# JARVIS-MoCap/JARVIS-HybridNet

Hardware: AMD Instinct MI355X
Metric: multi-view frames/s (12cam 1280x1024, 23kpt, 64^3 grid) (higher is better)
Workload: dtype f32; 1 GPU; BASELINE configs[2]: HybridNet 12-camera 1280x1024, 23 kpts, 64^3 grid, small/small; cameras=12, joints=23, grid=64, streams=3, parallelism=single GPU, 3 time batches in flight on 3 HIP streams, hipgraph=False

## Files before the change

include/jarvis_hip.h:

```cpp
#ifndef JARVIS_HIP_H
#define JARVIS_HIP_H
#include <stdint.h>

#ifdef __cplusplus
extern "C" {
#endif

#define JH_ABI_VERSION 4

const char* jh_last_error(void);
int jh_abi_version(void);

#define JH_PRECISION_DEFAULT (-1)
#define JH_PRECISION_F32 0
#define JH_PRECISION_BF16X3 1
#define JH_PRECISION_BF16X3_WIDE 2
int jh_set_precision(int mode);
int jh_get_precision(void);

typedef struct jh_params jh_params;
int jh_params_create(jh_params** out);
int jh_params_set(jh_params* p, const char* key, const float* host, int64_t numel);
void jh_params_destroy(jh_params* p);

// ... 152 lines not shown
int jh_predictor_set_spread(jh_predictor* pr, int on);
int jh_predictor_get_spread(jh_predictor* pr, float* cov_dev, float* peak_dev, float* mass_dev, void* stream);
int jh_predictor_debug_v2v(jh_predictor* pr, float* out_dev, void* stream);

#define JH_FRAME_SURFACE  4
#define JH_FRAME_SENSOR   5
int jh_predictor_forward_images(jh_predictor* pr, const void* const* images_host, int n_images, int format,
                                const jh_yuv_surface* yuv, const jh_sensor_surface* sensor, const uint8_t* mask_dev,
                                float* points_dev, float* conf_dev, int32_t* valid_dev, void* stream);

typedef struct jh_subjects_params {
  int32_t max_subjects, max_peaks, nms_radius, min_views;
  float min_peak, max_error_px;
} jh_subjects_params;
int jh_subjects_params_check(const jh_subjects_params* params);
int jh_op_center_peaks(const float* heat_dev, int n, int hh, int wh, int cp, const jh_subjects_params* params,
                       float* peaks_dev, int32_t* count_dev, void* stream);
int jh_op_associate_subjects(const float* peaks_dev, int t, int cams, const float* cam_dev, const float* intr_dev,
                             const float* dist_dev, int calib_per_frame, const uint8_t* mask_dev, float sx2, float sy2,
                             const jh_subjects_params* params, float* centers_dev, int32_t* views_dev,
                             int32_t* members_dev, float* error_dev, void* stream);
int jh_predictor_detect_subjects(jh_predictor* pr, const void* frames_dev, const void* const* images_host, int n_images,
                                 int format, const jh_yuv_surface* yuv, const jh_sensor_surface* sensor,
                                 const uint8_t* mask_dev, const jh_subjects_params* params, float* centers_dev,
                                 int32_t* views_dev, int32_t* members_dev, float* error_dev,
                                 float* peaks_dev , void* stream);

typedef struct jh_track_params {
  int32_t max_subjects;
  int32_t max_missed;
// ... 136 lines not shown
```

jarvis-hybridnet_amd/_native.py:

```python
import ctypes
import math
import os
from typing import NamedTuple

import torch

_HERE = os.path.dirname(os.path.abspath(__file__))
LIB_PATH = os.environ.get("JH_LIBRARY_PATH") or os.path.join(_HERE, "libjarvis_hip.so")
_lib = None

c_void_p, c_int, c_float, c_int64 = ctypes.c_void_p, ctypes.c_int, ctypes.c_float, ctypes.c_int64
c_char_p = ctypes.c_char_p


class PredictorConfig(ctypes.Structure):
    _fields_ = [("num_cameras", ctypes.c_int32), ("num_joints", ctypes.c_int32),
                ("center_size", ctypes.c_int32), ("bbox", ctypes.c_int32),
                ("roi_cube_size", c_float), ("grid_spacing", c_float),
                ("center_model", ctypes.c_int32), ("kp_model", ctypes.c_int32),
                ("img_h", ctypes.c_int32), ("img_w", ctypes.c_int32),
                ("time_batch", ctypes.c_int32), ("time_batch_3d", ctypes.c_int32),
                ("cam_lo", ctypes.c_int32),
                ("cam_n", ctypes.c_int32), ("mean", c_float * 3), ("std", c_float * 3),
                ("precision", ctypes.c_int32)]
# ... 147 lines not shown
    "jh_predictor_forward_masked": (c_int, [c_void_p, c_void_p, c_int, c_void_p, c_void_p, c_void_p, c_void_p,
                                            c_void_p]),
    "jh_predictor_forward_images": (c_int, [c_void_p, ctypes.POINTER(c_void_p), c_int, c_int,
                                            ctypes.POINTER(YuvSurfaceStruct), ctypes.POINTER(SensorSurfaceStruct),
                                            c_void_p, c_void_p, c_void_p, c_void_p, c_void_p]),
    "jh_predictor2d_forward_images": (c_int, [c_void_p, ctypes.POINTER(c_void_p), c_int, c_int,
                                              ctypes.POINTER(YuvSurfaceStruct), ctypes.POINTER(SensorSurfaceStruct),
                                              c_void_p, c_void_p, c_void_p, c_void_p]),
    "jh_predictor_stage_keypoints_masked": (c_int, [c_void_p, c_void_p, c_int, c_void_p, c_void_p, c_void_p,
                                                    c_void_p]),
    "jh_predictor_stage_3d_masked": (c_int, [c_void_p, c_void_p, c_int, c_void_p, c_void_p, c_void_p, c_void_p,
                                             c_void_p]),
    "jh_predictor_debug_mask": (c_int, [c_void_p, c_void_p, c_void_p, c_void_p]),
    "jh_predictor_views2d": (c_int, [c_void_p, c_void_p, c_int] + [c_void_p] * 8),
    "jh_subjects_params_check": (c_int, [ctypes.POINTER(SubjectsParamsStruct)]),
    "jh_op_center_peaks": (c_int, [c_void_p, c_int, c_int, c_int, c_int, ctypes.POINTER(SubjectsParamsStruct), c_void_p,
                                   c_void_p, c_void_p]),
    "jh_op_associate_subjects": (c_int, [c_void_p, c_int, c_int, c_void_p, c_void_p, c_void_p, c_int, c_void_p,
                                         c_float, c_float, ctypes.POINTER(SubjectsParamsStruct), c_void_p, c_void_p,
                                         c_void_p, c_void_p, c_void_p]),
    "jh_predictor_detect_subjects": (c_int, [c_void_p, c_void_p, ctypes.POINTER(c_void_p), c_int, c_int,
                                             ctypes.POINTER(YuvSurfaceStruct), ctypes.POINTER(SensorSurfaceStruct),
                                             c_void_p, ctypes.POINTER(SubjectsParamsStruct), c_void_p, c_void_p,
                                             c_void_p, c_void_p, c_void_p, c_void_p]),
    "jh_track_params_check": (c_int, [ctypes.POINTER(TrackParamsStruct)]),
    "jh_op_track_reset": (c_int, [c_void_p, c_void_p]),
    "jh_op_track_subjects": (c_int, [c_void_p, c_void_p, c_void_p, c_void_p, c_int, c_int,
                                     ctypes.POINTER(TrackParamsStruct)] + [c_void_p] * 10),
    "jh_joints3d_params_check": (c_int, [ctypes.POINTER(Joints3dParamsStruct)]),
    "jh_op_joint_peaks_refine": (c_int, [c_void_p, c_int, c_int, c_int, c_int, c_void_p, c_int, c_int, c_void_p,
# ... 460 lines not shown
```

jarvis-hybridnet_amd/csrc/api.hip:

```cpp
#include <cstring>
#include <memory>
#include "../../include/jarvis_hip.h"
#include <cstdlib>
#include "nets.h"
#include "bifpn_node.h"
#include "views2d.h"
#include "subjects.h"
#include "joints3d.h"
#include "tracks.h"

namespace jh {
static thread_local std::string g_err;
void set_error(const std::string& msg) { g_err = msg; }
}

using namespace jh;

struct jh_params { ParamMap map; };
struct jh_efftrack { EffTrackPlan plan; };
struct jh_v2v { V2VPlan plan; };

namespace {

struct Scratch {
// ... 616 lines not shown
  pr->J = cfg->num_joints; pr->Jp = cpad(cfg->num_joints);
  pr->B = cfg->bbox; pr->Hh = cfg->bbox / 2; pr->hs = cfg->bbox / 2 + 2;
  pr->G = (int)(cfg->roi_cube_size / cfg->grid_spacing);
  pr->Gh = pr->G / 2;
  JH_REQUIRE(pr->T >= 1 && pr->C >= 1 && pr->C <= 64, "time batch / camera count");
  JH_REQUIRE(cfg->cam_lo >= 0 && cfg->cam_n >= 1 && cfg->cam_lo + cfg->cam_n <= pr->C, "camera range");
  JH_REQUIRE(pr->G % 4 == 0, "ROI_CUBE_SIZE / GRID_SPACING must be a multiple of 4");
  const int N = pr->T * pr->Cloc;
  const NodeBatchClass node_class = pr->T >= 8 ? NodeBatchClass::AtLeast8 : NodeBatchClass::Below8;
  const int norm_kb = node_class == NodeBatchClass::AtLeast8 && JH_ENV_KNOB("JH_NODE_ROWS") != 0 ? 64 : 0;
  PlanSetup setup;
  if (setup.init(&pr->cfg, node_class, norm_kb)) return 1;
  if (center_params) {
    pr->center = setup.efftrack();
    if (pr->center->build(center_params->map, "", cfg->center_model, 1, N, cfg->center_size,
                          cfg->center_size)) return 1;
  }
  pr->kp = setup.efftrack();
  if (pr->kp->build(hybrid_params->map, "effTrack.", cfg->kp_model, pr->J, N, pr->B, pr->B)) return 1;
  pr->v2v.reset(new V2VPlan());
  pr->v2v->precision = setup.precision;
  pr->v2v->norm_block_kb = norm_kb;
  if (pr->v2v->build(hybrid_params->map, "v2vNet.", pr->J, pr->T3, pr->G)) return 1;
  auto& m = pr->mem;
  const int T = pr->T, C = pr->C;
  if (m.get(reinterpret_cast<void**>(&pr->cam), (size_t)C * 12 * sizeof(float))) return 1;
  if (m.get(reinterpret_cast<void**>(&pr->intr), (size_t)C * 9 * sizeof(float))) return 1;
  if (m.get(reinterpret_cast<void**>(&pr->dist), (size_t)C * 5 * sizeof(float))) return 1;
  if (m.get(reinterpret_cast<void**>(&pr->det_all), (size_t)T * C * 3 * sizeof(float))) return 1;
  if (m.get(reinterpret_cast<void**>(&pr->c3f), (size_t)T * 3 * sizeof(float))) return 1;
  for (auto& cs : pr->cset) {
// ... 826 lines not shown

extern "C" {

int jh_predictor2d_create(const jh_params* center_params, const jh_params* kp_params,
                          const jh_predictor_config* cfg, jh_predictor2d** out) {
  JH_REQUIRE(center_params && kp_params && cfg && out, "bad argument");
  std::unique_ptr<jh_predictor2d> pr(new jh_predictor2d());
  pr->cfg = *cfg;
  pr->T = cfg->time_batch; pr->J = cfg->num_joints; pr->B = cfg->bbox;
  JH_REQUIRE(pr->T >= 1, "batch");
  JH_REQUIRE(cfg->img_w >= pr->B + 1 && cfg->img_h >= pr->B + 1, "image smaller than the bounding box");
  PlanSetup setup;
  if (setup.init(&pr->cfg, NodeBatchClass::ByLaunchSize, 0)) return 1;
  pr->center = setup.efftrack();
  if (pr->center->build(center_params->map, "", cfg->center_model, 1, pr->T, cfg->center_size,
                        cfg->center_size)) return 1;
  pr->kp = setup.efftrack();
  if (pr->kp->build(kp_params->map, "", cfg->kp_model, pr->J, pr->T, pr->B, pr->B)) return 1;
  if (pr->mem.get(reinterpret_cast<void**>(&pr->det), (size_t)pr->T * 3 * sizeof(float))) return 1;
  if (pr->mem.get(reinterpret_cast<void**>(&pr->chm), (size_t)pr->T * 2 * sizeof(int))) return 1;
  if (pr->mem.get(reinterpret_cast<void**>(&pr->valid), (size_t)pr->T * sizeof(int))) return 1;
  JH_CHECK_HIP(hipDeviceSynchronize());
  *out = pr.release();
  return 0;
}

void jh_predictor2d_destroy(jh_predictor2d* pr) { delete pr; }

static int forward2d_impl(jh_predictor2d* pr, const Call& call, int32_t* points_dev, float* conf_dev,
                          int32_t* valid_dev) {
  hipStream_t s = call.s;
// ... 221 lines not shown
               const float* w_host, const float* b_host, const float* x_dev, int n, int d, int h,
               int w, const float* gate_dev, int norm_act, float* y_dev, void* stream) {
  return op_conv_body(nd, kind, k, stride, pad, cin, cout, w_host, b_host, x_dev, n, d, h, w, gate_dev, norm_act,
                      nullptr, y_dev, static_cast<hipStream_t>(stream), "jh_op_conv");
}

int jh_op_conv_operand(int nd, int kind, int k, int stride, int pad, int cin, int cout,
                       const float* w_host, const float* b_host, const float* x_dev, int n, int d, int h,
                       int w, const float* gate_dev, const jh_op_operand* operand, float* y_dev, void* stream) {
  JH_REQUIRE(operand && w_host && x_dev && y_dev && n >= 1, "bad argument");
  JH_REQUIRE(operand->in_act >= ACT_NONE && operand->in_act <= ACT_SILU, "jh_op_conv_operand: in_act");
  JH_REQUIRE(operand->latency_class == 0 || operand->latency_class == 1, "jh_op_conv_operand: latency_class");
  JH_REQUIRE(!(gate_dev && operand->se_pool_host), "either a gate tensor or a gate recipe");
  return op_conv_body(nd, kind, k, stride, pad, cin, cout, w_host, b_host, x_dev, n, d, h, w, gate_dev, -1, operand,
                      y_dev, static_cast<hipStream_t>(stream), "jh_op_conv_operand");
}

int jh_op_se_gate(const double* pool_host, int n, int c, int squeeze, float inv_hw, const float* wr_host,
                  const float* br_host, const float* we_host, const float* be_host, float* gate_dev, void* stream) {
  hipStream_t s = static_cast<hipStream_t>(stream);
  JH_REQUIRE(gate_dev && n >= 1, "bad argument");
  Scratch sc;
  SeGate se;
  const int Cp = cpad(c);
  if (op_upload_se(sc, pool_host, n, c, Cp, squeeze, inv_hw, wr_host, br_host, we_host, be_host, &se)) return 1;
  float* gate = nullptr;
  if (sc.get(reinterpret_cast<void**>(&gate), (size_t)n * Cp * sizeof(float))) return 1;
  if (launch_se_gate(se.pool, n, c, Cp, squeeze, inv_hw, se.wr, se.br, se.we, se.be, gate, s)) return 1;
  JH_CHECK_HIP(hipMemcpy2DAsync(gate_dev, c * sizeof(float), gate, Cp * sizeof(float), c * sizeof(float), n,
                                hipMemcpyDeviceToDevice, s));
// ... 222 lines not shown
```

jarvis-hybridnet_amd/csrc/deconv_c1.hip:

```cpp
#include "jh_common.h"
#include "operand_load.h"

namespace jh {

constexpr int kDcTY = 8, kDcTX = 16, kDcPY = 10, kDcPX = 18;

__global__ __launch_bounds__(256) void deconv_c1_kernel(
    const float* __restrict__ x, const double* __restrict__ st, float inv_cnt, int in_act,
    const float* __restrict__ w , float* __restrict__ y, int H, int W, int Cp,
    int cout_p) {
  extern __shared__ __attribute__((aligned(16))) float sm[];
  const int S = Cp + 4;
  float* nrm = sm;
  float* tile = nrm + 2 * Cp;
  const int tid = threadIdx.x;
  const BlockId bid = xcd_block();
  const int tiles_x = (W + kDcTX - 1) / kDcTX;
  const int y0 = (bid.x / tiles_x) * kDcTY, x0 = (bid.x % tiles_x) * kDcTX;
  const int n = bid.y;
  const int q = Cp >> 2;

  for (int c = tid; c < Cp; c += 256) {
    float mean = 0.f, rstd = 1.f;
    if (st) {
      const NormCoef k = norm_coef_times_inv(st + ((size_t)n * Cp + c) * kStatW, inv_cnt);
      mean = k.mean;
      rstd = k.rstd;
    }
    nrm[c] = mean;
    nrm[Cp + c] = rstd;
  }
  __syncthreads();
  const float* xin = x + (size_t)n * H * W * Cp;
  {
    constexpr int NPX = kDcPY * kDcPX, ITERS = (NPX + 15) / 16, UB = ITERS;
    const int slot = tid >> 4;
   for (int cq0 = 0; cq0 < q; cq0 += 16) {
    const int lc4 = cq0 + (tid & 15);
    const bool cact = lc4 < q;
    float4 mu = make_float4(0.f, 0.f, 0.f, 0.f), rs = make_float4(1.f, 1.f, 1.f, 1.f);
    if (cact) {
      mu = *reinterpret_cast<const float4*>(nrm + lc4 * 4);
      rs = *reinterpret_cast<const float4*>(nrm + Cp + lc4 * 4);
    }
#pragma unroll
    for (int it0 = 0; it0 < ITERS; it0 += UB) {
      float4 v[UB];
      bool ok[UB];
#pragma unroll
      for (int u = 0; u < UB; ++u) {
        const int pix = (it0 + u) * 16 + slot;
        const int iy = y0 - 1 + pix / kDcPX, ix = x0 - 1 + pix % kDcPX;
        ok[u] = it0 + u < ITERS && pix < NPX && cact && iy >= 0 && iy < H && ix >= 0 && ix < W;
        v[u] = ok[u] ? *reinterpret_cast<const float4*>(xin + ((size_t)iy * W + ix) * Cp + lc4 * 4)
                     : make_float4(0.f, 0.f, 0.f, 0.f);
      }
#pragma unroll
      for (int u = 0; u < UB; ++u) {
        const int pix = (it0 + u) * 16 + slot;
        if (it0 + u < ITERS && pix < NPX && cact) {
          float4 x4 = v[u];
          if (ok[u]) x4 = act4(norm_sub4(x4, mu, rs), in_act);
          *reinterpret_cast<float4*>(tile + pix * S + lc4 * 4) = x4;
        }
      }
    }
   }
  }
  __syncthreads();

  const int py = __builtin_amdgcn_readfirstlane(tid >> 7);
  const int p = tid & 127;
  const int tm = p / kDcTX, tn = p % kDcTX;
  const int ra = py ? tm + 2 : tm + 1, ka = py ? 0 : 1;
  const int rb = py ? tm + 1 : tm, kb = py ? 2 : 3;
  const float* ta = tile + (ra * kDcPX + tn) * S;
  const float* tb = tile + (rb * kDcPX + tn) * S;
  const float* __restrict__ wa = w + ka * 4 * Cp;
  const float* __restrict__ wb = w + kb * 4 * Cp;
  float o0 = 0.f, o1 = 0.f;
  for (int c = 0; c < Cp; c += 4) {
    const float4 a0 = *reinterpret_cast<const float4*>(ta + c);
    const float4 a1 = *reinterpret_cast<const float4*>(ta + S + c);
    const float4 a2 = *reinterpret_cast<const float4*>(ta + 2 * S + c);
    const float4 b0 = *reinterpret_cast<const float4*>(tb + c);
    const float4 b1 = *reinterpret_cast<const float4*>(tb + S + c);
    const float4 b2 = *reinterpret_cast<const float4*>(tb + 2 * S + c);
    const float4 wa0 = *reinterpret_cast<const float4*>(wa + 0 * Cp + c);
    const float4 wa1 = *reinterpret_cast<const float4*>(wa + 1 * Cp + c);
    const float4 wa2 = *reinterpret_cast<const float4*>(wa + 2 * Cp + c);
    const float4 wa3 = *reinterpret_cast<const float4*>(wa + 3 * Cp + c);
    const float4 wb0 = *reinterpret_cast<const float4*>(wb + 0 * Cp + c);
    const float4 wb1 = *reinterpret_cast<const float4*>(wb + 1 * Cp + c);
    const float4 wb2 = *reinterpret_cast<const float4*>(wb + 2 * Cp + c);
    const float4 wb3 = *reinterpret_cast<const float4*>(wb + 3 * Cp + c);
#define JH_DOT4(acc, u, v) acc = fmaf(u.x, v.x, acc); acc = fmaf(u.y, v.y, acc); \
                           acc = fmaf(u.z, v.z, acc); acc = fmaf(u.w, v.w, acc);
    JH_DOT4(o0, a1, wa1) JH_DOT4(o0, a0, wa3) JH_DOT4(o0, b1, wb1) JH_DOT4(o0, b0, wb3)
    JH_DOT4(o1, a2, wa0) JH_DOT4(o1, a1, wa2) JH_DOT4(o1, b2, wb0) JH_DOT4(o1, b1, wb2)
#undef JH_DOT4
  }
  const int m = y0 + tm, nn = x0 + tn;
  if (m < H && nn < W) {
    float* dst = y + (((size_t)n * 2 * H + 2 * m + py) * 2 * W + 2 * nn) * cout_p;
    for (int o = 0; o < 2; ++o) {
      float* d = dst + o * cout_p;
      *reinterpret_cast<float4*>(d) = make_float4(o ? o1 : o0, 0.f, 0.f, 0.f);
      for (int c = 4; c < cout_p; c += 4) *reinterpret_cast<float4*>(d + c) = make_float4(0.f, 0.f, 0.f, 0.f);
    }
  }
}

int launch_deconv_c1(const Act& x, const double* stats, float inv_cnt, int in_act, const float* w,
                     const Act& y, hipStream_t s) {
  JH_REQUIRE(y.H == 2 * x.H && y.W == 2 * x.W && y.N == x.N && y.C == 1, "deconv_c1 shapes");
  const size_t lds = ((size_t)2 * x.Cp + (size_t)kDcPY * kDcPX * (x.Cp + 4)) * sizeof(float);
  JH_REQUIRE(lds <= 160 * 1024, "deconv_c1 tile does not fit LDS");
  static bool big = false;
  if (lds > 64 * 1024 && !big) {
    JH_CHECK_HIP(hipFuncSetAttribute(reinterpret_cast<const void*>(deconv_c1_kernel),
                                     hipFuncAttributeMaxDynamicSharedMemorySize, 160 * 1024));
    big = true;
  }
  const int tiles = ((x.H + kDcTY - 1) / kDcTY) * ((x.W + kDcTX - 1) / kDcTX);
  hipLaunchKernelGGL(deconv_c1_kernel, dim3(tiles, x.N), dim3(256), lds, s, x.p, stats, inv_cnt,
                     in_act, w, y.p, x.H, x.W, x.Cp, y.Cp);
  JH_CHECK_HIP(hipGetLastError());
  return 0;
}

}
```

jarvis-hybridnet_amd/csrc/geometry.hip:

```cpp
#include "jh_common.h"
#include "dlt.h"
#include "preprocess.h"
#include "views2d.h"
#include "subjects.h"
#include "nets.h"

namespace jh {

template <int SRC>
__global__ __launch_bounds__(256) void preprocess_resize_kernel(
    const void* __restrict__ frames, float* __restrict__ out, int N, int H, int W, int S,
    float sy, float sx, float3 mean, float3 stdv, const void* const* __restrict__ frames_cell, int per_image,
    SrcDesc<SRC> d) {
  if (frames_cell && !per_image) frames = *frames_cell;
  const size_t total = (size_t)N * S * S;
  for (size_t i = (size_t)blockIdx.x * blockDim.x + threadIdx.x; i < total;
       i += (size_t)gridDim.x * blockDim.x) {
    const int ox = (int)(i % S), oy = (int)((i / S) % S);
    int n = (int)(i / ((size_t)S * S));
    const void* base = image_base(frames, frames_cell, per_image, n);
    *reinterpret_cast<float4*>(out + i * 4) = resize_px<SRC>(base, n, oy, ox, H, W, sy, sx, mean, stdv, d);
  }
}

// ... 545 lines not shown
                         const unsigned char* mask, const float* pts3d, const Calib& cal, int* points2d,
                         float* conf2d, float* reproj, float* err, unsigned char* used, int T, int C, int J, int Jp,
                         int Hh, int Wh, int hw, hipStream_t s) {
  if (check_scan_shape(T * C, Hh, Wh, J, Jp)) return 1;
  if (calib_check(cal, C)) return 1;
  const ScanShape sh = joint_argmax_all_shape(T * C, Hh, Wh, Jp);
  hipLaunchKernelGGL(views2d_final_kernel, dim3(T * C), dim3(round_up(J, kWave)), 0, s, pmax, pidx, center_hm,
                     valid, mask, pts3d, cal.cam, cal.intr, cal.dist, cal.fs, points2d, conf2d, reproj, err, used, C, J,
                     Jp, sh.slices, Hh, Wh, hw);
  JH_CHECK_HIP(hipGetLastError());
  return 0;
}

__device__ __forceinline__ float softplus_f(float x) { return x > 20.f ? x : log1pf(expf(x)); }

constexpr int kSpreadSums = 10, kSpreadRound = 5;
__device__ __forceinline__ unsigned long long spread_key(float x, unsigned p) {
  const unsigned u = __float_as_uint(x);
  const unsigned k = (u & 0x80000000u) ? ~u : (u | 0x80000000u);
  return ((unsigned long long)k << 32) | (unsigned long long)(0xFFFFFFFFu - p);
}
__device__ __forceinline__ unsigned long long max_u64(unsigned long long a, unsigned long long b) {
  return a > b ? a : b;
}
__device__ __forceinline__ void spread_acc(double* s, float h, double di, double dj, double dk) {
  const double d = (double)h, hi = d * di, hj = d * dj, hk = d * dk;
  s[0] += d; s[1] += hi; s[2] += hj; s[3] += hk;
  s[4] += hi * di; s[5] += hi * dj; s[6] += hi * dk;
  s[7] += hj * dj; s[8] += hj * dk; s[9] += hk * dk;
}
// ... 1 lines not shown
template <bool SPREAD>
__global__ __launch_bounds__(256) void softargmax_partial_kernel(
    const float* __restrict__ x, double* __restrict__ partial, int* __restrict__ pmax,
    double* __restrict__ spart, unsigned long long* __restrict__ skey, int Gh, int Jp, int ppb) {
  extern __shared__ __attribute__((aligned(16))) float sm[];
  const int q = Jp >> 2, rows = 256 / q, tid = threadIdx.x;
  const bool active = tid < rows * q;
  const int c4 = tid % q, row = tid / q;
  const int t = blockIdx.y;
  const int P = Gh * Gh * Gh;
  const int p0 = blockIdx.x * ppb, p1 = min(P, p0 + ppb);
  float4 s0 = make_float4(0, 0, 0, 0), si = s0, sj = s0, sk = s0, mx = s0;
  [[maybe_unused]] double ds[SPREAD ? 4 : 1][SPREAD ? kSpreadSums : 1] = {};
  [[maybe_unused]] unsigned long long key[SPREAD ? 4 : 1] = {};
  if (active) {
    for (int p = p0 + row; p < p1; p += rows) {
      const float4 v = *reinterpret_cast<const float4*>(x + ((size_t)t * P + p) * Jp + c4 * 4);
      const float4 h = make_float4(softplus_f(v.x), softplus_f(v.y), softplus_f(v.z), softplus_f(v.w));
      const float fk = (float)(p % Gh), fj = (float)((p / Gh) % Gh), fi = (float)(p / (Gh * Gh));
      s0.x += h.x; s0.y += h.y; s0.z += h.z; s0.w += h.w;
      si.x += h.x * fi; si.y += h.y * fi; si.z += h.z * fi; si.w += h.w * fi;
      sj.x += h.x * fj; sj.y += h.y * fj; sj.z += h.z * fj; sj.w += h.w * fj;
      sk.x += h.x * fk; sk.y += h.y * fk; sk.z += h.z * fk; sk.w += h.w * fk;
      mx.x = fmaxf(mx.x, h.x); mx.y = fmaxf(mx.y, h.y); mx.z = fmaxf(mx.z, h.z); mx.w = fmaxf(mx.w, h.w);
      if constexpr (SPREAD) {
        const double di = (double)fi, dj = (double)fj, dk = (double)fk;
        spread_acc(ds[0], h.x, di, dj, dk);
        spread_acc(ds[1], h.y, di, dj, dk);
        spread_acc(ds[2], h.z, di, dj, dk);
        spread_acc(ds[3], h.w, di, dj, dk);
        key[0] = max_u64(key[0], spread_key(v.x, (unsigned)p));
        key[1] = max_u64(key[1], spread_key(v.y, (unsigned)p));
        key[2] = max_u64(key[2], spread_key(v.z, (unsigned)p));
        key[3] = max_u64(key[3], spread_key(v.w, (unsigned)p));
      }
    }
  }
  if (active) {
    float4* p = reinterpret_cast<float4*>(sm) + ((size_t)row * q + c4) * 5;
    p[0] = s0; p[1] = si; p[2] = sj; p[3] = sk; p[4] = mx;
  }
  __syncthreads();
  for (int i = tid; i < q * 4 * 5; i += 256) {
    const int comp = i & 3, v = (i >> 2) % 5, cq = (i >> 2) / 5;
    const int ch = cq * 4 + comp;
    if (v < 4) {
      float acc = 0.f;
      for (int r = 0; r < rows; ++r) acc += sm[(((size_t)r * q + cq) * 5 + v) * 4 + comp];
      exact_add(partial + (((size_t)t * Jp + ch) * 4 + v) * kLimbs, (double)acc);
    } else {
      float m = 0.f;
      for (int r = 0; r < rows; ++r) m = fmaxf(m, sm[(((size_t)r * q + cq) * 5 + v) * 4 + comp]);
      atomicMax(pmax + (size_t)t * Jp + ch, __float_as_int(m));
    }
  }
  if constexpr (SPREAD) {
    constexpr int W = kSpreadRound + 1;
    double* dm = reinterpret_cast<double*>(sm);
#pragma unroll
    for (int round = 0; round < kSpreadSums / kSpreadRound; ++round) {
      __syncthreads();
      if (active) {
#pragma unroll
// ... 96 lines not shown

int launch_softargmax(const float* x, const int* center3d, double* partial, int* pmax,
                      float* points, float* conf, float* heatmap_final, int T, int J, int Jp,
                      int Gh, float spacing, float roi, hipStream_t s, const SoftargmaxSpread* sp) {
  const int P = Gh * Gh * Gh;
  const int q = Jp / 4;
  JH_REQUIRE(q >= 1 && q <= 64 && J <= 256, "soft-argmax joint count");
  const int rows = 256 / q;
  const size_t pbytes = (size_t)T * Jp * 4 * kLimbs * sizeof(double), mbytes = (size_t)T * Jp * sizeof(int);
  if (reinterpret_cast<char*>(pmax) == reinterpret_cast<char*>(partial) + pbytes) {
    if (launch_zero(partial, pbytes + mbytes, s)) return 1;
  } else {
    if (launch_zero(partial, pbytes, s)) return 1;
    if (launch_zero(pmax, mbytes, s)) return 1;
  }
  const int ppb = rows * 8;
  dim3 grid((P + ppb - 1) / ppb, T);
  if (sp) {
    JH_REQUIRE(sp->sums && sp->key && sp->cov && sp->peak && sp->mass, "soft-argmax spread: null pointer");
    JH_REQUIRE(grid.x <= (1u << 13), "soft-argmax spread: more than 2^13 blocks per frame set");
    if (launch_zero(sp->sums, softargmax_spread_sums(T, Jp) * sizeof(double) +
                                  (size_t)T * Jp * sizeof(unsigned long long), s)) return 1;
    hipLaunchKernelGGL(softargmax_partial_kernel<true>, grid, dim3(256),
                       (size_t)rows * Jp * (kSpreadRound + 1) * sizeof(double), s, x, partial, pmax, sp->sums,
                       sp->key, Gh, Jp, ppb);
  } else {
    hipLaunchKernelGGL(softargmax_partial_kernel<false>, grid, dim3(256), (size_t)rows * q * 20 * sizeof(float),
                       s, x, partial, pmax, (double*)nullptr, (unsigned long long*)nullptr, Gh, Jp, ppb);
  }
  JH_CHECK_HIP(hipGetLastError());
  hipLaunchKernelGGL(softargmax_final_kernel, dim3(T), dim3(256), 0, s, partial, pmax, center3d,
// ... 346 lines not shown
```

jarvis-hybridnet_amd/csrc/nets.h:

```cpp
#pragma once
#include <deque>
#include <functional>
#include <map>
#include <string>
#include <vector>
#include "jh_common.h"
#include "conv_layer.h"
#include "node_layer.h"
#include "preprocess.h"

namespace jh {

int launch_reproject(const Calib& cal, const int* center3d, const int* center_hm, const float* heat, float2* coarse,
                     float* vol, int* idx_out, int T, int C, int G, float spacing, int hs, int Jp, int heat_pad,
                     int div255, const unsigned char* mask, hipStream_t s, const HeatLayout* layout = nullptr);
int launch_reproject_joint_masked(const Calib& cal, const int* center3d, const int* center_hm, const float* heat,
                                  float2* coarse, float* vol, int* idx_out, int T, int C, int G, float spacing, int hs,
                                  int J, int Jp, int heat_pad, int div255, const unsigned char* mask,
                                  const unsigned char* joint_mask, const JointSets& js, hipStream_t s,
                                  const HeatLayout* layout = nullptr);
int launch_preprocess_resize(const void* frames, const FrameSource& src, float* out, int N, int H, int W, int S,
                             const float* mean, const float* stdv, hipStream_t s,
                             const void* const* frames_cell = nullptr);
int launch_preprocess_crop(const void* frames, const FrameSource& src, const int* center_hm, float* out, int T,
// ... 27 lines not shown
                      int Gh, float spacing, float roi, hipStream_t s, const SoftargmaxSpread* spread = nullptr);

typedef std::map<std::string, std::vector<float>> ParamMap;

class Plan {
 public:
  ~Plan();
  int run(hipStream_t s);
  size_t launches() const { return ops_.size(); }
  size_t device_bytes() const { return bytes_; }
  int precision = precision_mode();
  int norm_block_kb = 0;

 protected:
  int alloc(void** p, size_t bytes);
  int new_act(int N, int D, int H, int W, int C, Act* out);
  size_t scratch(size_t doubles);
  int finish();
  double* sc(size_t off) const { return arena_ + off; }
  int upload(const std::vector<float>& host, float** dev);
  int get(const ParamMap& pm, const std::string& key, size_t numel, const float** out);

  struct Op { std::function<int(hipStream_t)> fn; std::string name; double flops, bytes; };
  std::vector<Op> ops_;
  void push(const std::string& name, double flops, double bytes, std::function<int(hipStream_t)> fn) {
    ops_.push_back(Op{std::move(fn), name, flops, bytes});
  }
  std::vector<void*> owned_;
  std::deque<ConvLayer> layers_;
  std::vector<ConvWeights> convs_;
  double* arena_ = nullptr;
// ... 6 lines not shown
               float in_inv = 0.f, int in_act = 0, const SeGate* se = nullptr, long se_pool_off = -1);
  void add_norm(const Act& x, size_t stats_off, int act, const float* r1, const float* r2,
                float* y, long pool_off, long r1_stats_off = -1);
};

struct Ref {
  Act a;
  long st = -1;
  float inv = 0.f;
  int act = 0;
};

class EffTrackPlan : public Plan {
 public:
  int build(const ParamMap& pm, const std::string& prefix, int size, int J, int N, int H, int W,
            bool want_res1 = false);
  bool stem_fusable = false;
  StemSource stem_src;
  void set_stem_traffic(double bytes);
  int stem_channels() const { return stem_ch_; }
  NodeBatchClass node_class = NodeBatchClass::ByLaunchSize;
  Act input;
  Act heat;
  Act res1;
  int J = 0;
  int stem_op_ = -1, stem_ch_ = 16;

 private:
  int mbconv(const ParamMap& pm, const std::string& p, int stage, int k, int stride, int cin,
             int cout, int expand, Ref* x, Ref* out);
  void materialise(Ref* x);
// ... 20 lines not shown
```

jarvis-hybridnet_amd/csrc/nets.hip:

```cpp
#include <cmath>
#include <cstring>
#include <cstdlib>
#include "nets.h"
#include "bifpn_node.h"

namespace jh {

Profiler& profiler() {
  static Profiler p;
  return p;
}
void Profiler::begin(const std::string& name, double flops, double bytes, hipStream_t s) {
  ProfRec r{name, flops, bytes, nullptr, nullptr, 0.f};
  (void)hipEventCreate(&r.e0);
  (void)hipEventCreate(&r.e1);
  (void)hipEventRecord(r.e0, s);
  recs.push_back(r);
}
void Profiler::end(hipStream_t s) { (void)hipEventRecord(recs.back().e1, s); }
int Profiler::finish() {
  JH_CHECK_HIP(hipDeviceSynchronize());
  for (auto& r : recs) {
    if (!r.e0) continue;
    JH_CHECK_HIP(hipEventElapsedTime(&r.ms, r.e0, r.e1));
// ... 4 lines not shown
  return 0;
}

Plan::~Plan() {
  for (void* p : owned_) (void)hipFree(p);
  for (auto& c : convs_) free_conv_weights(&c);
}

int Plan::alloc(void** p, size_t bytes) {
  JH_CHECK_HIP(hipMalloc(p, bytes));
  owned_.push_back(*p);
  bytes_ += bytes;
  return 0;
}

int Plan::new_act(int N, int D, int H, int W, int C, Act* out) {
  out->N = N; out->D = D; out->H = H; out->W = W; out->C = C; out->Cp = cpad(C);
  if (alloc(reinterpret_cast<void**>(&out->p), out->bytes())) return 1;
  JH_CHECK_HIP(hipMemset(out->p, 0, out->bytes()));
  return 0;
}

size_t Plan::scratch(size_t doubles) {
  const size_t off = arena_doubles_;
  arena_doubles_ += (doubles + 7) / 8 * 8;
  return off;
}

int Plan::finish() {
  if (arena_doubles_ == 0) arena_doubles_ = 8;
  return alloc(reinterpret_cast<void**>(&arena_), arena_doubles_ * sizeof(double));
}
// ... 276 lines not shown
    NodeArgs b = a;
    b.st[0] = s0 >= 0 ? sc((size_t)s0) : nullptr;
    b.st[1] = s1 >= 0 ? sc((size_t)s1) : nullptr;
    b.st[2] = s2 >= 0 ? sc((size_t)s2) : nullptr;
    b.stats = sc(st);
    return launch_bifpn_node(b, choice, s);
  });
  return 0;
}

void EffTrackPlan::set_stem_traffic(double bytes) {
  if (stem_op_ >= 0 && stem_op_ < (int)ops_.size()) ops_[stem_op_].bytes = bytes;
}

int EffTrackPlan::build(const ParamMap& pm, const std::string& pre, int size, int joints, int N,
                        int H, int W, bool want_res1) {
  JH_REQUIRE(size >= 0 && size < 3, "model size");
  JH_REQUIRE(H % 64 == 0 && W % 64 == 0, "image side must be a multiple of 64");
  const SizeSpec& ss = kSizes[size];
  J = joints;
  int stem, taps[3];
  std::vector<Block> blocks;
  trunk(size, &stem, &blocks, taps);

  if (new_act(N, 1, H, W, 3, &input)) return 1;
  input.Cp = 4;
  Ref x;
  if (new_act(N, 1, H / 2, W / 2, stem, &x.a)) return 1;
  size_t st = 0;
  const std::string bb = pre + "backbone_net.model.";
  JH_REQUIRE(stem == 16 || stem == 32, "stem channels");
// ... 103 lines not shown
        if (fnode("p7_w2", 2, in, m_dn2, p7_in, "conv7_down", &p7_out)) return 1;
      }
    }
    p3 = p3_out; p4 = p4_out; p5 = p5_out; p6 = p6_out; p7 = p7_out;
  }

  const float* wc = nullptr;
  if (get(pm, pre + "weights_cat", 3, &wc)) return 1;
  float w[3], sum = 0.f;
  for (int i = 0; i < 3; ++i) { w[i] = wc[i] > 20.f ? wc[i] : log1pf(expf(wc[i])); sum += w[i]; }
  for (int i = 0; i < 3; ++i) w[i] = w[i] / (sum + 0.0001f);
  const Ref hin[3] = {p3, p4, p5};
  const int hmodes[3] = {FUSE_SAME, FUSE_UP2, FUSE_UP4};
  Ref mid;
  if (node(pm, pre + "first_conv.", 3, hin, hmodes, w, ACT_NONE, p3.a, ss.head, &mid)) return 1;
  if (new_act(N, 1, mid.a.H * 2, mid.a.W * 2, J, &heat)) return 1;
  if (want_res1) {
    if (new_act(N, 1, mid.a.H, mid.a.W, J, &res1)) return 1;
    if (add_conv(pm, conv_desc(2, 3, 1, 1, ss.head, J), pre + "final_conv1.weight", "", false, mid.a,
                 res1, nullptr, false, nullptr, mid.st, mid.inv, ACT_NONE)) return 1;
  }
  if (add_conv(pm, deconv2d_k4s2p1_desc(ss.head, J), pre + "deconv1.weight", "", true, mid.a, heat,
               nullptr, false, nullptr, mid.st, mid.inv, ACT_NONE)) return 1;
  return finish();
}

int V2VPlan::res_block(const ParamMap& pm, const std::string& p, int c, const Act& x,
                       const float* extra, Act* out, long x_stats, size_t* raw_stats) {
  Act a;
  if (new_act(x.N, x.D, x.H, x.W, c, &a)) return 1;
  size_t s1 = 0, s2 = 0;
// ... 65 lines not shown
```

Before: 2184 multi-view frames/s.

## Retile single-channel deconv, store dense center heatmap, unroll soft-argmax loads

The single-output-channel deconv kernel gets a larger 32x16 tile with channel-chunked staging, register-prefetched loads overlapping compute, and four output rows per thread. Its LDS footprint is capped at 64KB so the large-LDS attribute path goes away. The center heatmap is now allocated with one dense channel instead of padded channels, which cuts write traffic, and a raw deconv test entry point is added. Separately, the soft-argmax kernel batches eight loads per thread, steps grid indices incrementally instead of dividing, and unrolls the row reduction.

```diff
diff --git a/include/jarvis_hip.h b/include/jarvis_hip.h
--- a/include/jarvis_hip.h
+++ b/include/jarvis_hip.h
@@ -190,6 +190,8 @@
   float min_peak, max_error_px;
 } jh_subjects_params;
 int jh_subjects_params_check(const jh_subjects_params* params);
+int jh_op_deconv_c1_raw(int cin, const float* w_host, const float* x_dev, int n, int h, int w, int cout_p,
+                        float* y_dev, void* stream);
 int jh_op_center_peaks(const float* heat_dev, int n, int hh, int wh, int cp, const jh_subjects_params* params,
                        float* peaks_dev, int32_t* count_dev, void* stream);
 int jh_op_associate_subjects(const float* peaks_dev, int t, int cams, const float* cam_dev, const float* intr_dev,
diff --git a/jarvis-hybridnet_amd/_native.py b/jarvis-hybridnet_amd/_native.py
--- a/jarvis-hybridnet_amd/_native.py
+++ b/jarvis-hybridnet_amd/_native.py
@@ -185,6 +185,7 @@
     "jh_predictor_debug_mask": (c_int, [c_void_p, c_void_p, c_void_p, c_void_p]),
     "jh_predictor_views2d": (c_int, [c_void_p, c_void_p, c_int] + [c_void_p] * 8),
     "jh_subjects_params_check": (c_int, [ctypes.POINTER(SubjectsParamsStruct)]),
+    "jh_op_deconv_c1_raw": (c_int, [c_int, c_void_p, c_void_p, c_int, c_int, c_int, c_int, c_void_p, c_void_p]),
     "jh_op_center_peaks": (c_int, [c_void_p, c_int, c_int, c_int, c_int, ctypes.POINTER(SubjectsParamsStruct), c_void_p,
                                    c_void_p, c_void_p]),
     "jh_op_associate_subjects": (c_int, [c_void_p, c_int, c_int, c_void_p, c_void_p, c_void_p, c_int, c_void_p,
diff --git a/jarvis-hybridnet_amd/csrc/api.hip b/jarvis-hybridnet_amd/csrc/api.hip
--- a/jarvis-hybridnet_amd/csrc/api.hip
+++ b/jarvis-hybridnet_amd/csrc/api.hip
@@ -654,7 +654,7 @@
   if (center_params) {
     pr->center = setup.efftrack();
     if (pr->center->build(center_params->map, "", cfg->center_model, 1, N, cfg->center_size,
-                          cfg->center_size)) return 1;
+                          cfg->center_size, false, true)) return 1;
   }
   pr->kp = setup.efftrack();
   if (pr->kp->build(hybrid_params->map, "effTrack.", cfg->kp_model, pr->J, N, pr->B, pr->B)) return 1;
@@ -1511,7 +1511,7 @@
   if (setup.init(&pr->cfg, NodeBatchClass::ByLaunchSize, 0)) return 1;
   pr->center = setup.efftrack();
   if (pr->center->build(center_params->map, "", cfg->center_model, 1, pr->T, cfg->center_size,
-                        cfg->center_size)) return 1;
+                        cfg->center_size, false, true)) return 1;
   pr->kp = setup.efftrack();
   if (pr->kp->build(kp_params->map, "", cfg->kp_model, pr->J, pr->T, pr->B, pr->B)) return 1;
   if (pr->mem.get(reinterpret_cast<void**>(&pr->det), (size_t)pr->T * 3 * sizeof(float))) return 1;
@@ -1763,6 +1763,24 @@
   JH_REQUIRE(!(gate_dev && operand->se_pool_host), "either a gate tensor or a gate recipe");
   return op_conv_body(nd, kind, k, stride, pad, cin, cout, w_host, b_host, x_dev, n, d, h, w, gate_dev, -1, operand,
                       y_dev, static_cast<hipStream_t>(stream), "jh_op_conv_operand");
+}
+
+int jh_op_deconv_c1_raw(int cin, const float* w_host, const float* x_dev, int n, int h, int w, int cout_p,
+                        float* y_dev, void* stream) {
+  hipStream_t s = static_cast<hipStream_t>(stream);
+  JH_REQUIRE(w_host && x_dev && y_dev && n >= 1 && h >= 1 && w >= 1 && cin >= 1 && cout_p >= 1, "bad argument");
+  Scratch sc;
+  Act x;
+  if (sc.act(n, 1, h, w, cin, &x)) return 1;
+  Act y = x;
+  y.H = 2 * h; y.W = 2 * w; y.C = 1; y.Cp = cout_p; y.p = y_dev;
+  const std::vector<float> wt = taps_major(w_host, cin, 16, x.Cp);
+  float* wd = nullptr;
+  if (op_upload(sc, wt.data(), wt.size(), &wd)) return 1;
+  if (launch_to_channel_last(x_dev, x, s)) return 1;
+  if (launch_deconv_c1(x, nullptr, 0.f, ACT_NONE, wd, y, s)) return 1;
+  JH_CHECK_HIP(hipStreamSynchronize(s));
+  return 0;
 }
 
 int jh_op_se_gate(const double* pool_host, int n, int c, int squeeze, float inv_hw, const float* wr_host,
diff --git a/jarvis-hybridnet_amd/csrc/deconv_c1.hip b/jarvis-hybridnet_amd/csrc/deconv_c1.hip
--- a/jarvis-hybridnet_amd/csrc/deconv_c1.hip
+++ b/jarvis-hybridnet_amd/csrc/deconv_c1.hip
@@ -3,14 +3,18 @@
 
 namespace jh {
 
-constexpr int kDcTY = 8, kDcTX = 16, kDcPY = 10, kDcPX = 18;
+constexpr int kDcTY = 32, kDcTX = 16, kDcPY = kDcTY + 2, kDcPX = kDcTX + 2;
+constexpr int kDcChunk = 16;
+constexpr int kDcS = kDcChunk + 4;
+constexpr int kDcNPX = kDcPY * kDcPX;
+constexpr int kDcSlots = 256 / (kDcChunk / 4);
+constexpr int kDcIters = (kDcNPX + kDcSlots - 1) / kDcSlots;
 
 __global__ __launch_bounds__(256) void deconv_c1_kernel(
     const float* __restrict__ x, const double* __restrict__ st, float inv_cnt, int in_act,
     const float* __restrict__ w , float* __restrict__ y, int H, int W, int Cp,
     int cout_p) {
   extern __shared__ __attribute__((aligned(16))) float sm[];
-  const int S = Cp + 4;
   float* nrm = sm;
   float* tile = nrm + 2 * Cp;
   const int tid = threadIdx.x;
@@ -30,83 +34,95 @@
     nrm[c] = mean;
     nrm[Cp + c] = rstd;
   }
-  __syncthreads();
   const float* xin = x + (size_t)n * H * W * Cp;
-  {
-    constexpr int NPX = kDcPY * kDcPX, ITERS = (NPX + 15) / 16, UB = ITERS;
-    const int slot = tid >> 4;
-   for (int cq0 = 0; cq0 < q; cq0 += 16) {
-    const int lc4 = cq0 + (tid & 15);
-    const bool cact = lc4 < q;
-    float4 mu = make_float4(0.f, 0.f, 0.f, 0.f), rs = make_float4(1.f, 1.f, 1.f, 1.f);
-    if (cact) {
-      mu = *reinterpret_cast<const float4*>(nrm + lc4 * 4);
-      rs = *reinterpret_cast<const float4*>(nrm + Cp + lc4 * 4);
-    }
+  const int quad = tid & 3, slot = tid >> 2;
+  int off[kDcIters];
 #pragma unroll
-    for (int it0 = 0; it0 < ITERS; it0 += UB) {
-      float4 v[UB];
-      bool ok[UB];
+  for (int u = 0; u < kDcIters; ++u) {
+    const int pix = u * kDcSlots + slot;
+    const int iy = y0 - 1 + pix / kDcPX, ix = x0 - 1 + pix % kDcPX;
+    off[u] = (pix < kDcNPX && iy >= 0 && iy < H && ix >= 0 && ix < W) ? (iy * W + ix) * Cp : -1;
+  }
+  float4 v[kDcIters];
+  const auto request = [&](int chunk) {
+    const int lc4 = chunk * (kDcChunk / 4) + quad;
 #pragma unroll
-      for (int u = 0; u < UB; ++u) {
-        const int pix = (it0 + u) * 16 + slot;
-        const int iy = y0 - 1 + pix / kDcPX, ix = x0 - 1 + pix % kDcPX;
-        ok[u] = it0 + u < ITERS && pix < NPX && cact && iy >= 0 && iy < H && ix >= 0 && ix < W;
-        v[u] = ok[u] ? *reinterpret_cast<const float4*>(xin + ((size_t)iy * W + ix) * Cp + lc4 * 4)
-                     : make_float4(0.f, 0.f, 0.f, 0.f);
-      }
+    for (int u = 0; u < kDcIters; ++u)
+      v[u] = (lc4 < q && off[u] >= 0) ? *reinterpret_cast<const float4*>(xin + off[u] + lc4 * 4)
+                                      : make_float4(0.f, 0.f, 0.f, 0.f);
+  };
+  const auto stage = [&](int chunk) {
+    const int lc4 = chunk * (kDcChunk / 4) + quad;
+    if (lc4 >= q) return;
+    const float4 mu = *reinterpret_cast<const float4*>(nrm + lc4 * 4);
+    const float4 rs = *reinterpret_cast<const float4*>(nrm + Cp + lc4 * 4);
 #pragma unroll
-      for (int u = 0; u < UB; ++u) {
-        const int pix = (it0 + u) * 16 + slot;
-        if (it0 + u < ITERS && pix < NPX && cact) {
-          float4 x4 = v[u];
-          if (ok[u]) x4 = act4(norm_sub4(x4, mu, rs), in_act);
-          *reinterpret_cast<float4*>(tile + pix * S + lc4 * 4) = x4;
-        }
+    for (int u = 0; u < kDcIters; ++u) {
+      const int pix = u * kDcSlots + slot;
+      if (pix < kDcNPX) {
+        float4 x4 = v[u];
+        if (off[u] >= 0) x4 = act4(norm_sub4(x4, mu, rs), in_act);
+        *reinterpret_cast<float4*>(tile + pix * kDcS + quad * 4) = x4;
       }
     }
-   }
+  };
+
+  const int tm = tid / kDcTX, tn = tid % kDcTX;
+  const float* t0 = tile + ((2 * tm) * kDcPX + tn) * kDcS;
+  float o[8] = {0.f, 0.f, 0.f, 0.f, 0.f, 0.f, 0.f, 0.f};
+  const int chunks = (q + kDcChunk / 4 - 1) / (kDcChunk / 4);
+  request(0);
+  __syncthreads();
+  for (int chunk = 0; chunk < chunks; ++chunk) {
+    stage(chunk);
+    __syncthreads();
+    if (chunk + 1 < chunks) request(chunk + 1);
+    const int nq = min(kDcChunk / 4, q - chunk * (kDcChunk / 4));
+    for (int lq = 0; lq < nq; ++lq) {
+      float4 r[4][3];
+#pragma unroll
+      for (int i = 0; i < 4; ++i)
+#pragma unroll
+        for (int j = 0; j < 3; ++j)
+          r[i][j] = *reinterpret_cast<const float4*>(t0 + (i * kDcPX + j) * kDcS + lq * 4);
+      const float* __restrict__ wc = w + (chunk * (kDcChunk / 4) + lq) * 4;
+#define JH_DC1_W(ky, kx) (*reinterpret_cast<const float4*>(wc + ((ky) * 4 + (kx)) * Cp))
+#define JH_DC1_DOT4(acc, u, wv) { const float4 w4 = wv; acc = fmaf(u.x, w4.x, acc); acc = fmaf(u.y, w4.y, acc); \
+                                  acc = fmaf(u.z, w4.z, acc); acc = fmaf(u.w, w4.w, acc); }
+#define JH_DC1_ROW(oi, a, ka, b, kb)                                                              \
+      JH_DC1_DOT4(o[oi], r[a][1], JH_DC1_W(ka, 1)) JH_DC1_DOT4(o[oi], r[a][0], JH_DC1_W(ka, 3))           \
+      JH_DC1_DOT4(o[oi], r[b][1], JH_DC1_W(kb, 1)) JH_DC1_DOT4(o[oi], r[b][0], JH_DC1_W(kb, 3))           \
+      JH_DC1_DOT4(o[oi + 1], r[a][2], JH_DC1_W(ka, 0)) JH_DC1_DOT4(o[oi + 1], r[a][1], JH_DC1_W(ka, 2))   \
+      JH_DC1_DOT4(o[oi + 1], r[b][2], JH_DC1_W(kb, 0)) JH_DC1_DOT4(o[oi + 1], r[b][1], JH_DC1_W(kb, 2))
+      JH_DC1_ROW(0, 1, 1, 0, 3)
+      JH_DC1_ROW(2, 2, 0, 1, 2)
+      JH_DC1_ROW(4, 2, 1, 1, 3)
+      JH_DC1_ROW(6, 3, 0, 2, 2)
+#undef JH_DC1_ROW
+#undef JH_DC1_DOT4
+#undef JH_DC1_W
+    }
+    __syncthreads();
   }
-  __syncthreads();
-
-  const int py = __builtin_amdgcn_readfirstlane(tid >> 7);
-  const int p = tid & 127;
-  const int tm = p / kDcTX, tn = p % kDcTX;
-  const int ra = py ? tm + 2 : tm + 1, ka = py ? 0 : 1;
-  const int rb = py ? tm + 1 : tm, kb = py ? 2 : 3;
-  const float* ta = tile + (ra * kDcPX + tn) * S;
-  const float* tb = tile + (rb * kDcPX + tn) * S;
-  const float* __restrict__ wa = w + ka * 4 * Cp;
-  const float* __restrict__ wb = w + kb * 4 * Cp;
-  float o0 = 0.f, o1 = 0.f;
-  for (int c = 0; c < Cp; c += 4) {
-    const float4 a0 = *reinterpret_cast<const float4*>(ta + c);
-    const float4 a1 = *reinterpret_cast<const float4*>(ta + S + c);
-    const float4 a2 = *reinterpret_cast<const float4*>(ta + 2 * S + c);
-    const float4 b0 = *reinterpret_cast<const float4*>(tb + c);
-    const float4 b1 = *reinterpret_cast<const float4*>(tb + S + c);
-    const float4 b2 = *reinterpret_cast<const float4*>(tb + 2 * S + c);
-    const float4 wa0 = *reinterpret_cast<const float4*>(wa + 0 * Cp + c);
-    const float4 wa1 = *reinterpret_cast<const float4*>(wa + 1 * Cp + c);
-    const float4 wa2 = *reinterpret_cast<const float4*>(wa + 2 * Cp + c);
-    const float4 wa3 = *reinterpret_cast<const float4*>(wa + 3 * Cp + c);
-    const float4 wb0 = *reinterpret_cast<const float4*>(wb + 0 * Cp + c);
-    const float4 wb1 = *reinterpret_cast<const float4*>(wb + 1 * Cp + c);
-    const float4 wb2 = *reinterpret_cast<const float4*>(wb + 2 * Cp + c);
-    const float4 wb3 = *reinterpret_cast<const float4*>(wb + 3 * Cp + c);
-#define JH_DOT4(acc, u, v) acc = fmaf(u.x, v.x, acc); acc = fmaf(u.y, v.y, acc); \
-                           acc = fmaf(u.z, v.z, acc); acc = fmaf(u.w, v.w, acc);
-    JH_DOT4(o0, a1, wa1) JH_DOT4(o0, a0, wa3) JH_DOT4(o0, b1, wb1) JH_DOT4(o0, b0, wb3)
-    JH_DOT4(o1, a2, wa0) JH_DOT4(o1, a1, wa2) JH_DOT4(o1, b2, wb0) JH_DOT4(o1, b1, wb2)
-#undef JH_DOT4
-  }
-  const int m = y0 + tm, nn = x0 + tn;
-  if (m < H && nn < W) {
-    float* dst = y + (((size_t)n * 2 * H + 2 * m + py) * 2 * W + 2 * nn) * cout_p;
-    for (int o = 0; o < 2; ++o) {
-      float* d = dst + o * cout_p;
-      *reinterpret_cast<float4*>(d) = make_float4(o ? o1 : o0, 0.f, 0.f, 0.f);
-      for (int c = 4; c < cout_p; c += 4) *reinterpret_cast<float4*>(d + c) = make_float4(0.f, 0.f, 0.f, 0.f);
+  const int m = y0 + 2 * tm, nn = x0 + tn;
+  if (nn >= W) return;
+#pragma unroll
+  for (int ro = 0; ro < 4; ++ro) {
+    if (m + (ro >> 1) >= H) break;
+    float* d = y + (((size_t)n * 2 * H + 2 * m + ro) * 2 * W + 2 * nn) * cout_p;
+    const float a = o[2 * ro], b = o[2 * ro + 1];
+    if (cout_p == 1) {
+      *reinterpret_cast<float2*>(d) = make_float2(a, b);
+    } else if ((cout_p & 3) == 0) {
+      for (int px = 0; px < 2; ++px, d += cout_p) {
+        *reinterpret_cast<float4*>(d) = make_float4(px ? b : a, 0.f, 0.f, 0.f);
+        for (int c = 4; c < cout_p; c += 4) *reinterpret_cast<float4*>(d + c) = make_float4(0.f, 0.f, 0.f, 0.f);
+      }
+    } else {
+      for (int px = 0; px < 2; ++px, d += cout_p) {
+        d[0] = px ? b : a;
+        for (int c = 1; c < cout_p; ++c) d[c] = 0.f;
+      }
     }
   }
 }
@@ -114,14 +130,9 @@
 int launch_deconv_c1(const Act& x, const double* stats, float inv_cnt, int in_act, const float* w,
                      const Act& y, hipStream_t s) {
   JH_REQUIRE(y.H == 2 * x.H && y.W == 2 * x.W && y.N == x.N && y.C == 1, "deconv_c1 shapes");
-  const size_t lds = ((size_t)2 * x.Cp + (size_t)kDcPY * kDcPX * (x.Cp + 4)) * sizeof(float);
-  JH_REQUIRE(lds <= 160 * 1024, "deconv_c1 tile does not fit LDS");
-  static bool big = false;
-  if (lds > 64 * 1024 && !big) {
-    JH_CHECK_HIP(hipFuncSetAttribute(reinterpret_cast<const void*>(deconv_c1_kernel),
-                                     hipFuncAttributeMaxDynamicSharedMemorySize, 160 * 1024));
-    big = true;
-  }
+  JH_REQUIRE(y.Cp >= 1 && x.Cp % 8 == 0 && (long long)x.H * x.W * x.Cp < (1ll << 31), "deconv_c1 layout");
+  const size_t lds = ((size_t)2 * x.Cp + (size_t)kDcNPX * kDcS) * sizeof(float);
+  JH_REQUIRE(lds <= 64 * 1024, "deconv_c1 tile does not fit LDS");
   const int tiles = ((x.H + kDcTY - 1) / kDcTY) * ((x.W + kDcTX - 1) / kDcTX);
   hipLaunchKernelGGL(deconv_c1_kernel, dim3(tiles, x.N), dim3(256), lds, s, x.p, stats, inv_cnt,
                      in_act, w, y.p, x.H, x.W, x.Cp, y.Cp);
diff --git a/jarvis-hybridnet_amd/csrc/geometry.hip b/jarvis-hybridnet_amd/csrc/geometry.hip
--- a/jarvis-hybridnet_amd/csrc/geometry.hip
+++ b/jarvis-hybridnet_amd/csrc/geometry.hip
@@ -583,6 +583,7 @@
 
 __device__ __forceinline__ float softplus_f(float x) { return x > 20.f ? x : log1pf(expf(x)); }
 
+constexpr int kSoftUnroll = 8;
 constexpr int kSpreadSums = 10, kSpreadRound = 5;
 __device__ __forceinline__ unsigned long long spread_key(float x, unsigned p) {
   const unsigned u = __float_as_uint(x);
@@ -614,10 +615,28 @@
   [[maybe_unused]] double ds[SPREAD ? 4 : 1][SPREAD ? kSpreadSums : 1] = {};
   [[maybe_unused]] unsigned long long key[SPREAD ? 4 : 1] = {};
   if (active) {
-    for (int p = p0 + row; p < p1; p += rows) {
-      const float4 v = *reinterpret_cast<const float4*>(x + ((size_t)t * P + p) * Jp + c4 * 4);
+    float4 vv[kSoftUnroll];
+    const float* xt = x + (size_t)t * P * Jp + c4 * 4;
+#pragma unroll
+    for (int u = 0; u < kSoftUnroll; ++u) {
+      const int p = p0 + row + u * rows;
+      vv[u] = p < p1 ? *reinterpret_cast<const float4*>(xt + (size_t)p * Jp) : make_float4(0.f, 0.f, 0.f, 0.f);
+    }
+    const int pf = p0 + row;
+    int vi = pf / (Gh * Gh), vj = (pf / Gh) % Gh, vk = pf % Gh;
+    const int di = rows / (Gh * Gh), dj = (rows / Gh) % Gh, dk = rows % Gh;
+#pragma unroll
+    for (int u = 0; u < kSoftUnroll; ++u) {
+      const int p = pf + u * rows;
+      if (p >= p1) break;
+      const float4 v = vv[u];
       const float4 h = make_float4(softplus_f(v.x), softplus_f(v.y), softplus_f(v.z), softplus_f(v.w));
-      const float fk = (float)(p % Gh), fj = (float)((p / Gh) % Gh), fi = (float)(p / (Gh * Gh));
+      const float fk = (float)vk, fj = (float)vj, fi = (float)vi;
+      vk += dk;
+      if (vk >= Gh) { vk -= Gh; ++vj; }
+      vj += dj;
+      if (vj >= Gh) { vj -= Gh; ++vi; }
+      vi += di;
       s0.x += h.x; s0.y += h.y; s0.z += h.z; s0.w += h.w;
       si.x += h.x * fi; si.y += h.y * fi; si.z += h.z * fi; si.w += h.w * fi;
       sj.x += h.x * fj; sj.y += h.y * fj; sj.z += h.z * fj; sj.w += h.w * fj;
@@ -646,7 +665,17 @@
     const int ch = cq * 4 + comp;
     if (v < 4) {
       float acc = 0.f;
-      for (int r = 0; r < rows; ++r) acc += sm[(((size_t)r * q + cq) * 5 + v) * 4 + comp];
+      const float* col = sm + ((size_t)cq * 5 + v) * 4 + comp;
+      const int rs = q * 20;
+      int r = 0;
+      for (; r + 8 <= rows; r += 8) {
+        float e[8];
+#pragma unroll
+        for (int k = 0; k < 8; ++k) e[k] = col[(size_t)(r + k) * rs];
+#pragma unroll
+        for (int k = 0; k < 8; ++k) acc += e[k];
+      }
+      for (; r < rows; ++r) acc += col[(size_t)r * rs];
       exact_add(partial + (((size_t)t * Jp + ch) * 4 + v) * kLimbs, (double)acc);
     } else {
       float m = 0.f;
@@ -773,7 +802,7 @@
     if (launch_zero(partial, pbytes, s)) return 1;
     if (launch_zero(pmax, mbytes, s)) return 1;
   }
-  const int ppb = rows * 8;
+  const int ppb = rows * kSoftUnroll;
   dim3 grid((P + ppb - 1) / ppb, T);
   if (sp) {
     JH_REQUIRE(sp->sums && sp->key && sp->cov && sp->peak && sp->mass, "soft-argmax spread: null pointer");
diff --git a/jarvis-hybridnet_amd/csrc/nets.h b/jarvis-hybridnet_amd/csrc/nets.h
--- a/jarvis-hybridnet_amd/csrc/nets.h
+++ b/jarvis-hybridnet_amd/csrc/nets.h
@@ -65,7 +65,7 @@
 
  protected:
   int alloc(void** p, size_t bytes);
-  int new_act(int N, int D, int H, int W, int C, Act* out);
+  int new_act(int N, int D, int H, int W, int C, Act* out, int Cp = 0);
   size_t scratch(size_t doubles);
   int finish();
   double* sc(size_t off) const { return arena_ + off; }
@@ -102,7 +102,7 @@
 class EffTrackPlan : public Plan {
  public:
   int build(const ParamMap& pm, const std::string& prefix, int size, int J, int N, int H, int W,
-            bool want_res1 = false);
+            bool want_res1 = false, bool dense_heat = false);
   bool stem_fusable = false;
   StemSource stem_src;
   void set_stem_traffic(double bytes);
diff --git a/jarvis-hybridnet_amd/csrc/nets.hip b/jarvis-hybridnet_amd/csrc/nets.hip
--- a/jarvis-hybridnet_amd/csrc/nets.hip
+++ b/jarvis-hybridnet_amd/csrc/nets.hip
@@ -42,8 +42,8 @@
   return 0;
 }
 
-int Plan::new_act(int N, int D, int H, int W, int C, Act* out) {
-  out->N = N; out->D = D; out->H = H; out->W = W; out->C = C; out->Cp = cpad(C);
+int Plan::new_act(int N, int D, int H, int W, int C, Act* out, int Cp) {
+  out->N = N; out->D = D; out->H = H; out->W = W; out->C = C; out->Cp = Cp ? Cp : cpad(C);
   if (alloc(reinterpret_cast<void**>(&out->p), out->bytes())) return 1;
   JH_CHECK_HIP(hipMemset(out->p, 0, out->bytes()));
   return 0;
@@ -350,7 +350,7 @@
 }
 
 int EffTrackPlan::build(const ParamMap& pm, const std::string& pre, int size, int joints, int N,
-                        int H, int W, bool want_res1) {
+                        int H, int W, bool want_res1, bool dense_heat) {
   JH_REQUIRE(size >= 0 && size < 3, "model size");
   JH_REQUIRE(H % 64 == 0 && W % 64 == 0, "image side must be a multiple of 64");
   const SizeSpec& ss = kSizes[size];
@@ -484,7 +484,8 @@
   const int hmodes[3] = {FUSE_SAME, FUSE_UP2, FUSE_UP4};
   Ref mid;
   if (node(pm, pre + "first_conv.", 3, hin, hmodes, w, ACT_NONE, p3.a, ss.head, &mid)) return 1;
-  if (new_act(N, 1, mid.a.H * 2, mid.a.W * 2, J, &heat)) return 1;
+  JH_REQUIRE(!dense_heat || J == 1, "a dense heat map has one channel");
+  if (new_act(N, 1, mid.a.H * 2, mid.a.W * 2, J, &heat, dense_heat ? 1 : 0)) return 1;
   if (want_res1) {
     if (new_act(N, 1, mid.a.H, mid.a.W, J, &res1)) return 1;
     if (add_conv(pm, conv_desc(2, 3, 1, 1, ss.head, J), pre + "final_conv1.weight", "", false, mid.a,
```

New measurement: 2199 multi-view frames/s (median of 6 runs). No clear change (+0.7%).
